# techpro-studio/NNToolkitCore

Hardware: AMD Instinct MI355X
Metric: audio frames/sec (whole node) (higher is better)
Workload: dtype f32

## Files before the change

### nntoolkitcore_amd/csrc/hip/nntk_common.hpp

```cpp
#pragma once
#include <hip/hip_runtime.h>
#include <math.h>
#include "nntk_shim.h"

hipStream_t nntk_stream();
int nntk_fail(const char *what, hipError_t err);
int nntk_fail_msg(const char *what);
enum { NNTK_SPAN_REC = 0, NNTK_SPAN_SPEC = 1 };
int nntk_prof_span_begin(int kind);
void nntk_prof_span_end(int idx, long launches, long units);

struct NntkOptions {
    int rec_persistent = -1;
    int rec_xw = -1;
    int rec_pingpong = -1;
    int rec_groups = 2;
    int rec_spin_us = 1000000;
    int rec_stream = -1;
    int rec_fused2 = -1;
    int rec_rr = -1;
    int rec_xf = -1;
    int rec_fk = -1;
    int rec_hf = -1;
    int rec_bd = -1;
    int dense_frag3 = -1;
    int dense_f16x2 = -1;
    int train_outer_plain = -1;
    int train_bptt = -1;
    int spec_ppw = 0;
    int spec_variant = -1;
#ifdef NNTK_VARIANT_SPEC_DMA
    int spec_dma = -1;
#endif
    int bn_fast = 0;
    int gemm_tm_batch = -1;
    int conv_a4 = 1;
    int conv_flatk = -1;
    int conv_frag3_out = -1;
    int conv_store = -1;
    int gemm_split_bf16 = -1;
    int gemm_wide = -1;
    int conv_dbg = 0;
    int weights_check = -1;
};
const NntkOptions &nntk_options();

unsigned *nntk_fault_word();
int nntk_fault_enqueue_copy();
int nntk_persistent_disabled();
void nntk_persistent_launch_begin();
void nntk_persistent_launch_end();
bool nntk_weights_exact_only(const void *d_wp);
int nntk_cu_count();
void nntk_set_last_conv_kernel(const char *name);
void nntk_set_last_rec_kernel(const char *name);
int nntk_set_max_dynamic_lds(const void *kernel, size_t bytes);
// ... 54 lines not shown
```

### nntoolkitcore_amd/csrc/hip/recurrent_rr.hip

```cpp
#include "recurrent_rr_common.hpp"

__host__ __device__ inline int rr_blocks_per_ct(int KH, int KX) { return 4 * KH * 2 * 2 + 4 * KH * 2 + 4 * KX * 2 * 3; }

template <bool RAW>
__global__ __launch_bounds__(256) void rr_pack_kernel(const float *__restrict__ ut, const float *__restrict__ wp,
                                                      rr_v4u *__restrict__ img, int H, int in, int Hj_p, int Hk_p, int Kin_p,
                                                      int KH, int KX, int NCT, float uscale = 0.0f, float wscale = 1.0f) {
    const int bpc = rr_blocks_per_ct(KH, KX);
    const long total = (long)NCT * bpc * 64;
    for (long e = blockIdx.x * (long)blockDim.x + threadIdx.x; e < total; e += (long)gridDim.x * blockDim.x) {
        const int l = (int)(e & 63);
        const long blk = e >> 6;
        const int ct = (int)(blk / bpc);
        int r = (int)(blk % bpc);
        int part, w, i, mt, m;
        const int n_uh = 4 * KH * 4, n_ul = 4 * KH * 2;
        if (r < n_uh) { part = 0; m = r & 1; mt = (r >> 1) & 1; i = (r >> 2) % KH; w = (r >> 2) / KH; }
        else if (r < n_uh + n_ul) { r -= n_uh; part = 1; m = 2; mt = r & 1; i = (r >> 1) % KH; w = (r >> 1) / KH; }
        else { r -= n_uh + n_ul; part = 2; m = r % 3; mt = (r / 3) & 1; i = (r / 6) % KX; w = (r / 6) / KX; }
        const int c = 32 * mt + (l & 31);
        const int g = (c >> 3) & 3;
        const int j = 16 * ct + 8 * ((c >> 2) & 1) + 4 * (c >> 5) + (c & 3);
        const int ks = part == 2 ? w * KX + i : w * KH + i;
        float v[8];
// ... 20 lines not shown
                for (int q = 0; q < 4; ++q) rr_split_pair_f16(v[2 * q] * uscale, v[2 * q + 1] * uscale, h4[q], l4[q]);
                img[e] = m == 0 ? (rr_v4u){h4[0], h4[1], h4[2], h4[3]} : (rr_v4u){l4[0], l4[1], l4[2], l4[3]};
                continue;
            }
            if (part == 1) { img[e] = (rr_v4u){0u, 0u, 0u, 0u}; continue; }
#pragma unroll
            for (int q = 0; q < 8; ++q) v[q] *= wscale;
        }
        rr_split8(v, hi, mid, lo);
        img[e] = m == 0 ? hi : m == 1 ? mid : lo;
    }
}

__global__ __launch_bounds__(256) void rr_tile_h0_kernel(const float *__restrict__ h0, rr_v4u *__restrict__ hb, int B, int H, int NKS) {
    const long total = (long)((B + 63) / 64) * 2 * (H / 16) * 64;
    for (long e = blockIdx.x * (long)blockDim.x + threadIdx.x; e < total; e += (long)gridDim.x * blockDim.x) {
        const int l = (int)(e & 63);
        long r = e >> 6;
        const int ks = (int)(r % (H / 16)); r /= (H / 16);
        const int half = (int)(r & 1);
        const long bt = r >> 1;
        const long row = bt * 64 + half * 32 + (l & 31);
        if (row >= B) continue;
        float v[8];
#pragma unroll
        for (int q = 0; q < 8; ++q) v[q] = h0[row * H + 16 * ks + 8 * (l >> 5) + q];
        rr_v4u hi, mid, lo;
        rr_split8(v, hi, mid, lo);
        rr_v4u *dst = hb + ((((size_t)bt * 2 + half) * NKS + ks) * 3) * 64 + l;
        dst[0] = hi; dst[64] = mid; dst[128] = lo;
    }
}

template <int KH, int KX, bool TRAIN, int CELL, bool XF, bool HF = false, bool VL = false, bool BD = false>
__device__ __forceinline__ void rr_body(const RRParams &p) {
    static_assert(!VL || !HF, "VL: not with the two-f16-image hand-off");
    static_assert(!BD || (VL && XF), "BD: per-row lengths and a frag3 x operand");
    constexpr int NH = HF ? 2 : 3;
#ifndef RR_ULR8
#define RR_ULR8 0
#endif
    constexpr bool ULR = !HF && (KX > 2 || (RR_ULR8 && KH == 8 && !TRAIN));
    constexpr int NST = KX + KH;
#ifndef RR_S_RED
#define RR_S_RED 0
#endif
    constexpr int S_RED = (RR_S_RED) && KH == 8 ? 1 : 0, S_PUB = S_RED + 1;
    constexpr int S_XSPL = KX > 2 ? KX : S_PUB + 1;
#ifndef RR_PEND
#define RR_PEND (KH == 4)
#endif
    constexpr bool PEND = RR_PEND;
#ifndef RR_S_E1_XLATE
#define RR_S_E1_XLATE 2
#endif
#ifndef RR_HF_S_E1
#define RR_HF_S_E1 2
#endif
    constexpr int S_E1 = (KX > 2 ? RR_S_E1_XLATE : HF ? RR_HF_S_E1 : RR_S_E1) + S_RED;
    constexpr bool X_LATE = KX > 2;
    constexpr int S_E2 = NST - 1;
#ifndef RR_HEAD_LEAD
#define RR_HEAD_LEAD 1
#endif
    constexpr int S_HEAD = !PEND ? S_E2 : S_E2 - RR_HEAD_LEAD > S_PUB ? S_E2 - RR_HEAD_LEAD : S_PUB + 1;
#ifndef RR_HF_NPRE
#define RR_HF_NPRE 5
#endif
    constexpr int NPRE = (HF ? RR_HF_NPRE : RR_NPRE) < KH ? (HF ? RR_HF_NPRE : RR_NPRE) : KH;
    constexpr int own_lo = S_PUB + NPRE < KH ? S_PUB + NPRE : KH, own_hi = S_E1 + NPRE < KH ? S_E1 + NPRE : KH;
    constexpr int NXR = XF ? 3 * KX : 2 * KX;
    constexpr int N_X_AFTER_PUB = (X_LATE || S_XSPL >= S_E1) ? 0 : NXR;
    constexpr int N_AFTER_PUB = NH * (own_hi - own_lo) + N_X_AFTER_PUB;
    static_assert(!HF || (!PEND && !TRAIN && XF && CELL == 0 && !ULR), "HF: the flag-protocol LSTM instantiations with a frag3 x operand");
    static_assert(NST >= 5 && S_XSPL >= KX && S_XSPL > S_PUB && KH - NPRE <= S_E2 && S_HEAD > S_PUB && S_HEAD <= S_E2, "slice schedule");
#ifndef RR_POLL_LEAD_RR
#define RR_POLL_LEAD_RR (NST >= 9 ? 2 : RR_POLL_LEAD)
#endif
#ifndef RR_HF_POLL_LEAD
#define RR_HF_POLL_LEAD RR_POLL_LEAD_RR
#endif
    constexpr int POLL_LEAD = HF ? RR_HF_POLL_LEAD : RR_POLL_LEAD_RR;
    static_assert(PEND ? S_XSPL < S_E2 : (S_E1 < S_E2 && S_E1 > S_PUB && S_XSPL < S_E2 - POLL_LEAD), "slice schedule");
    extern __shared__ __attribute__((aligned(16))) char smem[];
    rr_v4u *ULs = reinterpret_cast<rr_v4u *>(smem);
    rr_v4u *WXs = ULs + ((ULR || HF) ? 0 : 4 * KH * 2 * 64);
    rr_v4u *red = WXs + 4 * KX * 6 * 64;
    float *hx = reinterpret_cast<float *>(red + 32 * 64);
    unsigned *hs = reinterpret_cast<unsigned *>(hx + 32 * RR_HX_LD);

    const int tid = threadIdx.x;
    const int lane = tid & 63;
    const int w = __builtin_amdgcn_readfirstlane(tid >> 6);
    const int n = lane & 31, kh = lane >> 5;
    const int bt = blockIdx.x % p.NBT;
    const int ct = blockIdx.x / p.NBT;
    const int bt_abs = p.b_base / 64 + bt;
    const int b0 = p.b_base + bt * 64;
    const int H = p.H;
    const int T = VL ? __builtin_amdgcn_readfirstlane(p.len[p.B + bt_abs]) : p.T;
    const int NKS = H >> 4;
    const bool bwd = BD && b0 >= p.bd_pad;
    const int rb0 = bwd ? b0 - p.bd_pad : b0;
    const int rows_valid = BD ? (p.bd_rows - rb0 < 64 ? p.bd_rows - rb0 : 64) : p.B - b0 < 64 ? p.B - b0 : 64;
    if (VL && T == 0) {
        if constexpr (BD) rr_bd_pass_state(p, b0, 64, 16 * ct, 16);
        else rr_vl_pass_state(p, b0, 64, 16 * ct, 16, CELL == 0);
// ... 187 lines not shown
                const float zg = nntk_fast_sigmoid(zc[0][e]);
                const float rg = nntk_fast_sigmoid(zc[1][e]);
                const float ht = nntk_fast_tanh(fmaf(rg, zc[2][e], zc[3][e]));
                hn[e] = fmaf(-zg + 1.0f, ht, zg * cst[half][e]);
                if constexpr (VL) hn[e] = t < vlen[half] ? hn[e] : cst[half][e];
                cst[half][e] = hn[e];
                if (TRAIN) {
                    zc[2][e] = fmaf(rg, zc[2][e], zc[3][e]);
                    zc[3][e] = z[2][e] + bsum[2][e];
                    ac[0][e] = zg; ac[1][e] = rg; ac[2][e] = ht;
                }
                continue;
            }
            const float ig = nntk_fast_sigmoid(zc[0][e]);
            const float fg = nntk_fast_sigmoid(zc[1][e]);
            const float gg = nntk_fast_tanh(zc[2][e]);
            const float og = nntk_fast_sigmoid(zc[3][e]);
            const float cn = fmaf(fg, cst[half][e], ig * gg);
            if constexpr (VL) {
                const bool live = t < vlen[half];
                hn[e] = live ? og * nntk_fast_tanh(cn) : hkeep[half][e];
                cst[half][e] = live ? cn : cst[half][e];
                hkeep[half][e] = hn[e];
            } else {
            cst[half][e] = cn;
            hn[e] = og * nntk_fast_tanh(cn);
            }
            ac[0][e] = ig; ac[1][e] = fg; ac[2][e] = gg; ac[3][e] = og;
        }
        *reinterpret_cast<float2 *>(hx + n * RR_HX_LD + jl) = make_float2(hn[0], hn[1]);
        if (HF && !RR_DBG(128)) {
            unsigned sh, sl;
            rr_split_pair_h2(hn[0], hn[1], sh, sl);
            unsigned *d = hs + n * RR_HS_LD + (jl >> 1);
            d[0] = sh; d[32 * RR_HS_LD] = sl;
        } else if (!RR_DBG(128)) {
            unsigned sh, sm, sl;
            rr_split_pair(hn[0], hn[1], sh, sm, sl);
            if (PEND) { sh = min(sh, 0xfffffffeu); sm = min(sm, 0xfffffffeu); sl = min(sl, 0xfffffffeu); }
            unsigned *d = hs + n * RR_HS_LD + (jl >> 1);
            d[0] = sh; d[32 * RR_HS_LD] = sm; d[2 * 32 * RR_HS_LD] = sl;
        }
        bool own_step = true;
        if constexpr (VL) own_step = t < vlen[half];
        if (TRAIN && CELL == 1) {
            const int row = b0 + half * 32 + n;
            if (row < p.B && jf + 1 < H + 1 && own_step) {
                float *zrow = p.z_cache + ((size_t)row * p.T + t) * 6 * H + jf;
#pragma unroll
                for (int g = 0; g < 3; ++g) {
                    *reinterpret_cast<float2 *>(zrow + g * H) = make_float2(zc[g][0], zc[g][1]);
                    *reinterpret_cast<float2 *>(zrow + (3 + g) * H) = make_float2(ac[g][0], ac[g][1]);
                }
                *reinterpret_cast<float2 *>(p.c_cache + ((size_t)row * p.T + t) * H + jf) = make_float2(zc[3][0], zc[3][1]);
            }
        } else if (TRAIN) {
            const int row = b0 + half * 32 + n;
            if (row < p.B && jf + 1 < H + 1 && own_step) {
                float *zrow = p.z_cache + ((size_t)row * p.T + t) * 8 * H + jf;
#pragma unroll
                for (int g = 0; g < 4; ++g) {
                    *reinterpret_cast<float2 *>(zrow + g * H) = make_float2(zc[g][0], zc[g][1]);
                    *reinterpret_cast<float2 *>(zrow + (4 + g) * H) = make_float2(ac[g][0], ac[g][1]);
                }
                *reinterpret_cast<float2 *>(p.c_cache + ((size_t)row * p.T + t) * H + jf) = make_float2(cst[half][0], cst[half][1]);
            }
// ... 35 lines not shown
                rr_v4u h2hi, h2lo;
                rr_split8_h2(v8, h2hi, h2lo);
                const __amdgpu_buffer_rsrc_t rs2 = __builtin_amdgcn_make_buffer_rsrc((void *)(p.out_h2 + (size_t)t * p.h2step), 0, (int)p.h2step, 0x00020000);
                const int vo = lane16 + (((bt_abs * 2 + half) * NKS + ct) * 2) * 1024;
                __builtin_amdgcn_raw_buffer_store_b128(h2hi, rs2, vo, 0, 0);
                __builtin_amdgcn_raw_buffer_store_b128(h2lo, rs2, vo + 1024, 0, 0);
                RR_BOUND(5, (size_t)t * p.h2step, vo + 1024, 0, p.h2step, 16);
            }
            if (BD && LAST) {
                int b0e = rb0;
                asm volatile("" : "+s"(b0e));
                const int row = b0e + half * 32 + n;
                if (row < p.bd_rows && !p.return_sequences) {
                    float *o = (bwd ? p.out_b : p.out) + (size_t)row * ldo + 16 * ct + 8 * kh;
                    *reinterpret_cast<rr_v4u *>(o) = o0; *reinterpret_cast<rr_v4u *>(o + 4) = o1;
                }
            } else if (LAST) {
                int b0e = b0;
                asm volatile("" : "+s"(b0e));
                const int row = b0e + half * 32 + n;
                if (row < p.B) {
                    if (!p.return_sequences && p.out) {
                        float *o = p.out + (size_t)row * H + 16 * ct + 8 * kh;
                        *reinterpret_cast<rr_v4u *>(o) = o0; *reinterpret_cast<rr_v4u *>(o + 4) = o1;
                    }
                    if (p.hT) {
                        float *o = p.hT + (size_t)row * H + 16 * ct + 8 * kh;
                        *reinterpret_cast<rr_v4u *>(o) = o0; *reinterpret_cast<rr_v4u *>(o + 4) = o1;
                    }
                }
            }
        } else if (PEND && w == ((2 * half + 2) & 3)) {
            if (!RR_DBG(128)) {
                const int vo = lane16 + (((bt_abs * 2 + half) * NKS + ct) * 3) * 1024;
                const __amdgpu_buffer_rsrc_t rs2 = rs_wr(t + 2 < T ? t + 2 : t);
                const int vo2 = t + 2 < T ? vo : RR_OOB_F;
                const rr_v4u pend = {RR_PENDING, RR_PENDING, RR_PENDING, RR_PENDING};
                __builtin_amdgcn_raw_buffer_store_b128(pend, rs2, vo2, 0, RR_ST_AUX);
                __builtin_amdgcn_raw_buffer_store_b128(pend, rs2, vo2 + 1024, 0, RR_ST_AUX);
                __builtin_amdgcn_raw_buffer_store_b128(pend, rs2, vo2 + 2048, 0, RR_ST_AUX);
                RR_BOUND(3, (size_t)(t + 2 < T ? t + 2 : t) * p.hstep, vo2 + 2048, 0, hb_bytes, 16);
            }
        }
    };
    unsigned *const flags0 = p.flags + (size_t)bt * 2 * RR_FLAGS, *const flags1 = flags0 + RR_FLAGS;
    auto arrive = [&](int half, int t, auto xlive_tag) __attribute__((always_inline)) {
        if (w == 2 * half) {
            asm volatile("s_waitcnt vmcnt(%0)" :: "i"(N_AFTER_PUB - (decltype(xlive_tag)::value ? 0 : N_X_AFTER_PUB)) : "memory");
            if (lane == 0)
                __hip_atomic_store((half ? flags1 : flags0) + ct, (unsigned)(t + 1), __ATOMIC_RELAXED, __HIP_MEMORY_SCOPE_AGENT);
        }
    };
    unsigned pv0 = 0;
    const bool flag_live = lane < p.NCT;
    auto poll_a = [&](int half) __attribute__((always_inline)) {
        const unsigned *f = (half ? flags1 : flags0) + lane;
        asm volatile("global_load_dword %0, %1, off sc1" : "=v"(pv0) : "v"(f) : "memory");
    };
    auto poll_b = [&](int half, int t) __attribute__((always_inline)) {
        asm volatile("s_waitcnt vmcnt(0)" : "+v"(pv0) :: "memory");
        const unsigned target = (unsigned)t;
        bool ok = !flag_live || pv0 >= target;
        if (__builtin_amdgcn_ballot_w64(!ok) != 0 || p.spin_ticks == 0) {
            const unsigned *f = (half ? flags1 : flags0) + lane;
            const unsigned long long t_start = __builtin_amdgcn_s_memrealtime();
            bool expired = p.spin_ticks == 0;
            while (!expired) {
                const unsigned a = __hip_atomic_load(f, __ATOMIC_RELAXED, __HIP_MEMORY_SCOPE_AGENT);
                ok = !flag_live || a >= target;
                if (__builtin_amdgcn_ballot_w64(!ok) == 0) break;
                if (__hip_atomic_load(p.fault, __ATOMIC_RELAXED, __HIP_MEMORY_SCOPE_AGENT) != 0) { expired = true; break; }
                __builtin_amdgcn_s_sleep(1);
                expired = __builtin_amdgcn_s_memrealtime() - t_start > p.spin_ticks;
            }
            if (expired && lane == 0) __hip_atomic_fetch_or(p.fault, 1u, __ATOMIC_RELAXED, __HIP_MEMORY_SCOPE_AGENT);
        }
    };

    auto probe_h = [&](auto half_tag, int i) __attribute__((always_inline)) {
        constexpr int half = decltype(half_tag)::value;
        unsigned mx = 0;
#pragma unroll
        for (int m = 0; m < 3; ++m) {
            const rr_v4u v = hf[half][i][m];
            mx = max(mx, max(max(v.x, v.y), max(v.z, v.w)));
        }
        return __builtin_amdgcn_ballot_w64(mx == RR_PENDING);
    };
    const unsigned long long inject = p.spin_ticks == 0 ? ~0ull : 0ull;
    auto settle_h = [&](auto half_tag, int t, int i, unsigned long long pend) __attribute__((always_inline)) {
        if (__builtin_expect((pend | inject) != 0, 0)) {
            const unsigned long long t_start = __builtin_amdgcn_s_memrealtime();
            bool expired = p.spin_ticks == 0;
            while (!expired) {
                issue_h(half_tag, t, 3 * i, 3 * i + 3);
                if (probe_h(half_tag, i) == 0) break;
                if (__hip_atomic_load(p.fault, __ATOMIC_RELAXED, __HIP_MEMORY_SCOPE_AGENT) != 0) { expired = true; break; }
                __builtin_amdgcn_s_sleep(1);
                expired = __builtin_amdgcn_s_memrealtime() - t_start > p.spin_ticks;
            }
            if (expired && lane == 0) __hip_atomic_fetch_or(p.fault, 1u, __ATOMIC_RELAXED, __HIP_MEMORY_SCOPE_AGENT);
        }
    };

    auto exchange = [&](const f32x16 (&acc)[2], int d0, int d1) __attribute__((always_inline)) {
        if (RR_DBG(32)) return;
#pragma unroll
        for (int dst = 0; dst < 4; ++dst) {
            if (dst < d0 || dst >= d1) continue;
            const int mt = dst >> 1, o = 2 * (dst & 1);
            const rr_v4u q0 = {__float_as_uint(acc[mt][o]), __float_as_uint(acc[mt][o + 1]), __float_as_uint(acc[mt][4 + o]), __float_as_uint(acc[mt][5 + o])};
            const rr_v4u q1 = {__float_as_uint(acc[mt][8 + o]), __float_as_uint(acc[mt][9 + o]), __float_as_uint(acc[mt][12 + o]), __float_as_uint(acc[mt][13 + o])};
            red[((dst * 4 + w) * 2 + 0) * 64 + lane] = q0;
            red[((dst * 4 + w) * 2 + 1) * 64 + lane] = q1;
        }
    };
    auto half_step = [&](auto y_tag, auto fin_tag, auto next_tag, auto poll_tag, auto last_tag, auto xlive_tag, int t, int tX) __attribute__((always_inline)) {
        constexpr bool XLIVE = decltype(xlive_tag)::value;
        constexpr int Y = decltype(y_tag)::value;
        using XT = std::integral_constant<int, 1 - Y>;
        constexpr int X = 1 - Y;
        constexpr bool FIN = decltype(fin_tag)::value, NEXT = decltype(next_tag)::value, POLL = decltype(poll_tag)::value;
        constexpr bool YCHK = PEND;
        f32x16 acc[2];
        unsigned long long pend_next = 0;
#pragma unroll
        for (int mt = 0; mt < 2; ++mt)
#pragma unroll
// ... 8 lines not shown
                for (int mt = 0; mt < 2; ++mt)
#pragma unroll
                    for (int m = 0; m < 3; ++m)
                        wa[mt][m] = __builtin_bit_cast(rr_bf16x8, WXs[((((w * KX + s) * 2 + mt) * 3) + m) * 64 + lane]);
            } else if (ULR) {
#pragma unroll
                for (int mt = 0; mt < 2; ++mt) ulo[mt] = ulr[s - KX][mt];
            } else if (HF) {
            } else {
#pragma unroll
                for (int mt = 0; mt < 2; ++mt)
                    ulo[mt] = ULPRE ? ulo_n[mt]
                                    : __builtin_bit_cast(rr_bf16x8, ULs[((w * KH + (s - KX)) * 2 + mt) * 64 + lane]);
            }
            if (s == S_RED && FIN && !RR_DBG(2)) { fin_reduce(); fin_gates(XT{}, tX); }
            if (s == S_PUB && FIN && !RR_DBG(2)) { fin_publish(XT{}, last_tag, tX); }
            if (!PEND) {
                if (s == S_E1 && FIN && !RR_DBG(4)) { arrive(X, tX, xlive_tag); }
                if (s == S_E2 - POLL_LEAD && NEXT && POLL && !RR_DBG(4)) poll_a(X);
                if (s == S_E2 && NEXT && POLL && !RR_DBG(4)) poll_b(X, tX + 1);
            }
            if (s == S_HEAD && NEXT && !RR_DBG(1)) issue_h(XT{}, tX + 1, 0, NH * NPRE);
            if (s == S_E2 && X_LATE && XLIVE && !RR_DBG(8)) issue_x(y_tag, t + 1);
            if (s + NPRE < KH && !RR_DBG(1)) issue_h(y_tag, t, NH * (s + NPRE), NH * (s + NPRE + 1));
            if (RR_DBG(16)) {
            } else if (s < KX) {
#pragma unroll
                for (int pr = 0; pr < 6; ++pr)
#pragma unroll
                    for (int mt = 0; mt < 2; ++mt)
                        acc[mt] = __builtin_amdgcn_mfma_f32_32x32x16_bf16(wa[mt][PA[pr]], xf[XF ? Y : 0][s][PB[pr]], acc[mt], 0, 0, 0);
            } else {
                const int i = s - KX;
                if (YCHK && t > 0 && !RR_DBG(4) && !RR_DBG(1)) settle_h(y_tag, t, i, pend_next);
                if constexpr (HF) {
                    constexpr int QA[3] = {0, 1, 0}, QB[3] = {1, 0, 0};
                    rr_f16x8 bh[2];
#pragma unroll
                    for (int m = 0; m < 2; ++m) bh[m] = __builtin_bit_cast(rr_f16x8, hf[Y][i][m]);
                    if (s == NST - 1) {
#pragma unroll
                        for (int mt = 0; mt < 2; ++mt) {
#pragma unroll
                            for (int pr = 0; pr < 3; ++pr)
                                acc[mt] = __builtin_amdgcn_mfma_f32_32x32x16_f16(__builtin_bit_cast(rr_f16x8, uh[i][mt][QA[pr]]), bh[QB[pr]], acc[mt], 0, 0, 0);
                            if (mt == 0) exchange(acc, 0, 2);
                        }
                    } else {
#pragma unroll
                        for (int pr = 0; pr < 3; ++pr)
#pragma unroll
                            for (int mt = 0; mt < 2; ++mt)
                                acc[mt] = __builtin_amdgcn_mfma_f32_32x32x16_f16(__builtin_bit_cast(rr_f16x8, uh[i][mt][QA[pr]]), bh[QB[pr]], acc[mt], 0, 0, 0);
                    }
                } else {
                rr_bf16x8 b[3];
#pragma unroll
                for (int m = 0; m < 3; ++m) b[m] = __builtin_bit_cast(rr_bf16x8, hf[Y][i][m]);
                if (s == NST - 1) {
#pragma unroll
                    for (int mt = 0; mt < 2; ++mt) {
#pragma unroll
                        for (int pr = 0; pr < 6; ++pr) {
                            const rr_bf16x8 av = PA[pr] == 2 ? ulo[mt] : uh[i][mt][PA[pr]];
                            acc[mt] = __builtin_amdgcn_mfma_f32_32x32x16_bf16(av, b[PB[pr]], acc[mt], 0, 0, 0);
                        }
                        if (mt == 0) exchange(acc, 0, 2);
                    }
                } else {
#pragma unroll
                for (int pr = 0; pr < 6; ++pr)
#pragma unroll
                    for (int mt = 0; mt < 2; ++mt) {
                        const rr_bf16x8 av = PA[pr] == 2 ? ulo[mt] : uh[i][mt][PA[pr]];
                        acc[mt] = __builtin_amdgcn_mfma_f32_32x32x16_bf16(av, b[PB[pr]], acc[mt], 0, 0, 0);
                    }
                }
                }
            }
            if (YCHK && s + 1 >= KX && s + 1 < NST && !RR_DBG(4) && !RR_DBG(1)) pend_next = probe_h(y_tag, s + 1 - KX);
            if (ULPRE && s + 1 >= KX && s + 1 < NST) {
#pragma unroll
                for (int mt = 0; mt < 2; ++mt) ulo_n[mt] = __builtin_bit_cast(rr_bf16x8, ULs[((w * KH + (s + 1 - KX)) * 2 + mt) * 64 + lane]);
            }
            if (s == S_XSPL) {
                if (NEXT && !RR_DBG(8)) split_x();
                if (!X_LATE && XLIVE && !RR_DBG(8)) issue_x(y_tag, t + 1);
            }
#ifndef RR_NO_INTERLEAVE
#ifdef RR_VALU_IL
#pragma unroll
            for (int j = 0; j < 12; ++j) {
                __builtin_amdgcn_sched_group_barrier(0x008, 1, 0);
                __builtin_amdgcn_sched_group_barrier(0x002, RR_VALU_IL, 0);
                if (j & 1) __builtin_amdgcn_sched_group_barrier(0x010, 1, 0);
            }
#else
            if (s == NST - 1) {
#pragma unroll
                for (int j = 0; j < 3; ++j) {
                    __builtin_amdgcn_sched_group_barrier(0x008, 2, 0);
                    __builtin_amdgcn_sched_group_barrier(0x010, 1, 0);
                }
#pragma unroll
                for (int j = 0; j < 4; ++j) {
                    __builtin_amdgcn_sched_group_barrier(0x008, 1, 0);
                    __builtin_amdgcn_sched_group_barrier(0x200, 1, 0);
                    __builtin_amdgcn_sched_group_barrier(0x010, 1, 0);
                }
                __builtin_amdgcn_sched_group_barrier(0x008, 2, 0);
            } else {
#pragma unroll
            for (int j = 0; j < 6; ++j) {
// ... 9 lines not shown
        exchange(acc, 2, 4);
    };

    issue_x(I0{}, 0);
    issue_h(I0{}, 0, 0, NH * NPRE);
    split_x();
    issue_x(I1{}, 0);
    if (T > 1) {
        half_step(I0{}, Ff{}, Tt{}, Ff{}, Ff{}, Tt{}, 0, -1);
        half_step(I1{}, Tt{}, Tt{}, Tt{}, Ff{}, Tt{}, 0, 0);
        for (int t = 1; t < T - 1; ++t) {
            half_step(I0{}, Tt{}, Tt{}, Tt{}, Ff{}, Tt{}, t, t - 1);
            half_step(I1{}, Tt{}, Tt{}, Tt{}, Ff{}, Tt{}, t, t);
        }
        half_step(I0{}, Tt{}, Tt{}, Tt{}, Ff{}, Ff{}, T - 1, T - 2);
    } else {
        half_step(I0{}, Ff{}, Tt{}, Ff{}, Ff{}, Ff{}, 0, -1);
    }
    half_step(I1{}, Tt{}, Ff{}, Ff{}, Tt{}, Ff{}, T - 1, T - 1);
    fin_reduce();
    fin_gates(I1{}, T - 1);
    fin_publish(I1{}, Tt{}, T - 1);
    int b0e = b0;
    asm volatile("" : "+s"(b0e));
#pragma unroll
    for (int half = 0; half < 2; ++half) {
        const int row = b0e + half * 32 + n;
        if (p.cT && row < p.B) {
            if (jf < H) p.cT[(size_t)row * H + jf] = cst[half][0];
            if (jf + 1 < H) p.cT[(size_t)row * H + jf + 1] = cst[half][1];
        }
    }
}
template <int KH, int KX, bool TRAIN = false, bool XF = false, bool HF = false, bool VL = false, bool BD = false>
__global__ __launch_bounds__(256) void lstm_rr_kernel(RRParams p) { rr_body<KH, KX, TRAIN, 0, XF, HF, VL, BD>(p); }
template <int KH, int KX, bool TRAIN = false, bool XF = false, bool VL = false, bool BD = false>
__global__ __launch_bounds__(256) void gru_rr_kernel(RRParams p) { rr_body<KH, KX, TRAIN, 1, XF, false, VL, BD>(p); }

#ifdef NNTK_RR_BOUNDS
static unsigned long long *g_rr_bounds = nullptr;
extern "C" int nntk_shim_rr_bounds_fetch(unsigned long long out[8]) {
    for (int i = 0; i < 8; ++i) out[i] = 0;
    if (!g_rr_bounds) return 0;
    if (hipDeviceSynchronize() != hipSuccess) return -1;
    if (hipMemcpy(out, g_rr_bounds, 64, hipMemcpyDeviceToHost) != hipSuccess) return -1;
    (void)hipMemset(g_rr_bounds, 0, 64);
    return 0;
}
#endif
static bool rr_shape(int H, int in, bool xf, int *KH, int *KX) {
    if (H < 64 || H > 512 || (H % 16) != 0 || in < 1) return false;
    if (!xf && (in < 8 || (in % 8) != 0)) return false;
    *KH = H <= 256 ? 4 : 8;
    *KX = in <= 64 ? 1 : in <= 128 ? 2 : (in <= 256 && *KH == 4) ? 4 : 0;
    return *KX != 0;
}
static bool rr_shape_hf(int H, int in, int *KH, int *KX) {
    if (H <= 256 || H > 512 || (H % 16) != 0 || in < 1) return false;
    *KH = 8;
    *KX = in <= 64 ? 1 : in <= 128 ? 2 : in <= 256 ? 4 : 0;
    return *KX != 0;
}
static size_t rr_lds_bytes(int KH, int KX, bool train = false, bool hf = false) {
    const bool ulr = hf || KX > 2 || (RR_ULR8 && KH == 8 && !train);
    return (size_t)((ulr ? 0 : 4 * KH * 2) + 4 * KX * 6 + 32) * 1024 + 32 * RR_HX_LD * 4 + 3 * 32 * RR_HS_LD * 4;
}
static size_t rr_step_bytes(int B, int H) { return (size_t)((B + 63) / 64) * 2 * (H / 16) * 3 * 1024; }

// ... 153 lines not shown
}

static int rr_launch(const RRIo &io, const float *d_img, const float *d_bi, const float *d_bh,
                     int B, int T, int in, int H, int return_sequences, int cell) {
    if (B <= 0 || T <= 0) return 0;
    const bool xf = io.xf3 != nullptr;
    const bool train = io.c_cache != nullptr;
    if (xf && (train || io.x_tm)) return 1;
    const bool vl = io.len != nullptr;
    if (vl && (io.x_tm || io.out_tm || io.hf || io.out_h2)) return nntk_fail_msg("lstm_rr: lengths with a stacked / frag2h call");
    const bool bd = io.out_b != nullptr;
    if (bd && (!vl || !xf || io.h0 || io.hT || io.cT)) return nntk_fail_msg("lstm_rr: a bidirectional call needs lengths, a frag3 x and no carried state");
    if (!xf && !io.x) return nntk_fail_msg("lstm_rr: no input");
    if (!io.hseq || !io.work) return nntk_fail_msg("lstm_rr: no hand-off buffer");
    if (io.x_tm && (double)T * B * in * 4 >= 2.0e9) return 1;
    if (io.out_tm && (!return_sequences || !io.out || (double)T * B * H * 4 >= 2.0e9)) return 1;
    if (io.out_h2 && (io.out || io.img4 || train || !return_sequences)) return nntk_fail_msg("lstm_rr: frag2h output with an f32 output / on the full-K family");
    const NntkOptions &opt = nntk_options();
    if (opt.rec_rr == 0 || opt.rec_persistent == 0 || nntk_persistent_disabled()) return 1;
    int KH, KX;
    const bool hf = io.hf != 0;
    if (!(hf ? rr_shape_hf(H, in, &KH, &KX) : rr_shape(H, in, xf, &KH, &KX))) return 1;
    if (!xf && ((((size_t)io.x) & 15) != 0 || (in % 4) != 0)) return 1;
    if (hf && (KH != 8 || cell != 0 || !xf || train || io.h0 || io.out || io.out_h2 || io.img4 || !return_sequences || opt.rec_hf == 0)) return 1;
    const int NCT = H / 16;
    if (!rr_tile_fits(T, in, bd ? io.ldo : H)) return 1;
    void (*kern)(RRParams) = nullptr;
    if (KH == 8 && KX == 2) kern = rr_pick<8, 2>(cell, train, xf, vl, bd);
    else if (KH == 8 && KX == 1) kern = rr_pick<8, 1>(cell, train, xf, vl, bd);
    else if (KH == 4 && KX == 4) kern = rr_pick<4, 4>(cell, train, xf, vl, bd);
    else if (KH == 4 && KX == 2) kern = rr_pick<4, 2>(cell, train, xf, vl, bd);
    else if (KH == 4 && KX == 1) kern = rr_pick<4, 1>(cell, train, xf, vl, bd);
    if (hf) kern = KX == 4 ? lstm_rr_kernel<8, 4, false, true, true> : KX == 2 ? lstm_rr_kernel<8, 2, false, true, true> : lstm_rr_kernel<8, 1, false, true, true>;
    if (!kern) return 1;
    const size_t lds = rr_lds_bytes(KH, KX, train, hf);
    if (lds > 160 * 1024) return 1;
    if (nntk_set_max_dynamic_lds((const void *)kern, lds)) return -1;
    const int resident = nntk_resident_blocks((const void *)kern, 256, lds, 1);
    const int tiles_per_launch = resident / NCT;
    if (tiles_per_launch < 1) return 1;
    unsigned *fault = nntk_fault_word();
    if (!fault) return 1;
    const size_t step = hf ? rr_step_bytes(B, H) / 3 * 2 : rr_step_bytes(B, H);
    if (step >= (size_t)RR_OOB_F) return 1;
    const int nbt_total = (B + 63) / 64;
    const size_t xstep = (size_t)nbt_total * 2 * ((in + 15) / 16) * 3 * 1024;
    if (xf && xstep >= (size_t)RR_OOB_F) return 1;
    unsigned *flags = reinterpret_cast<unsigned *>(io.work + step / 4);
    if (nntk_shim_memset(io.work, 0, step + (size_t)((B + 127) / 128) * 4 * RR_FLAGS * sizeof(unsigned))) return -1;
    if (nntk_shim_memset(io.hseq, 0xff, step * (size_t)(T < 2 ? T : 2))) return -1;
    if (io.h0) {
        long g = ((long)nbt_total * 2 * NCT * 64 + 255) / 256;
        if (g > 2048) g = 2048;
        hipLaunchKernelGGL(rr_tile_h0_kernel, dim3((unsigned)g), dim3(256), 0, nntk_stream(), io.h0, (rr_v4u *)io.work, B, H, H / 16);
    }
    RRParams q;
    q.x = io.x; q.img = (const rr_v4u *)d_img; q.bi = d_bi; q.bh = d_bh;
    q.h0f = (char *)io.work; q.hseq = (char *)io.hseq; q.hstep = step;
    q.xf3 = (const char *)io.xf3; q.xstep = xstep; q.NKSx = (in + 15) / 16;
    q.c0 = io.c0; q.cT = io.cT; q.hT = io.hT; q.out = io.out;
    q.c_cache = io.c_cache; q.z_cache = io.z_cache;
    q.x_tm = io.x_tm; q.out_tm = io.out_tm;
    q.fault = fault;
    q.spin_ticks = (unsigned long long)(opt.rec_spin_us > 0 ? opt.rec_spin_us : 0) * 100ull;
    q.B = B; q.T = T; q.H = H; q.in = in; q.NCT = NCT; q.return_sequences = return_sequences;
    q.NHT = nbt_total * 2;
    q.out_h2 = (char *)io.out_h2; q.h2step = rr_step_bytes(B, H) / 3 * 2;
    q.z_scale = io.z_scale;
    q.len = io.len; q.h0 = io.h0;
    q.img_b = (const rr_v4u *)io.img_b; q.bi_b = io.bi_b; q.bh_b = io.bh_b; q.out_b = io.out_b;
    q.bd_pad = bd ? B / 2 : 0; q.bd_rows = io.bd_rows; q.ldo = io.ldo;
#ifdef NNTK_REC_STAMPS
    q.stamp = nullptr;
    const char *stamp_path = getenv("NNTK_REC_STAMP_FILE");
    if (stamp_path) {
        if (hipMalloc((void **)&q.stamp, (size_t)(T + 1) * 64 * 8) != hipSuccess) return nntk_fail_msg("stamp alloc");
        (void)hipMemset(q.stamp, 0, (size_t)(T + 1) * 64 * 8);
    }
#endif
#ifdef NNTK_RR_BOUNDS
    static unsigned long long *g_bounds = nullptr;
    if (!g_bounds) {
// ... 9 lines not shown
    int took4 = 1;
    if (xf && !train && io.img4 && !io.out_tm) {
        q.flags = flags;
        took4 = nntk_fk_launch(q, io.img4, io.img4_b, cell, &launches);
        if (took4 < 0) { nntk_persistent_launch_end(); return -1; }
    }
    if (took4 == 1)
    for (int bt0 = 0; bt0 < nbt_total; bt0 += tiles_per_launch) {
        const int nbt = nbt_total - bt0 < tiles_per_launch ? nbt_total - bt0 : tiles_per_launch;
        q.NBT = nbt; q.b_base = bt0 * 64;
        q.flags = flags + (size_t)bt0 * 2 * RR_FLAGS;
        hipLaunchKernelGGL(kern, dim3((unsigned)(nbt * NCT)), dim3(256), lds, nntk_stream(), q);
    }
    const int copy_rc = nntk_fault_enqueue_copy();
    nntk_persistent_launch_end();
    if (copy_rc) return -1;
    nntk_prof_span_end(span, (long)launches, T);
#ifdef NNTK_REC_STAMPS
    if (q.stamp) {
        (void)hipStreamSynchronize(nntk_stream());
        unsigned long long *hs = (unsigned long long *)malloc((size_t)(T + 1) * 64 * 8);
        (void)hipMemcpy(hs, q.stamp, (size_t)(T + 1) * 64 * 8, hipMemcpyDeviceToHost);
        FILE *f = fopen(stamp_path, "wb");
        if (f) { fwrite(hs, 8, (size_t)(T + 1) * 64, f); fclose(f); }
        free(hs); (void)hipFree(q.stamp);
    }
#endif
    NNTK_LAUNCH_CHECK("lstm_rr_kernel");
    static const char *const names[2][2][3] = {{{"lstm_rr_kernel<4,1>", "lstm_rr_kernel<4,2>", "lstm_rr_kernel<4,4>"}, {"lstm_rr_kernel<8,1>", "lstm_rr_kernel<8,2>", ""}},
                                               {{"gru_rr_kernel<4,1>", "gru_rr_kernel<4,2>", "gru_rr_kernel<4,4>"}, {"gru_rr_kernel<8,1>", "gru_rr_kernel<8,2>", ""}}};
    static const char *const bd_names[2][2][3] = {{{"lstm_rr_kernel<4,1,bd>", "lstm_rr_kernel<4,2,bd>", "lstm_rr_kernel<4,4,bd>"}, {"lstm_rr_kernel<8,1,bd>", "lstm_rr_kernel<8,2,bd>", ""}},
                                                  {{"gru_rr_kernel<4,1,bd>", "gru_rr_kernel<4,2,bd>", "gru_rr_kernel<4,4,bd>"}, {"gru_rr_kernel<8,1,bd>", "gru_rr_kernel<8,2,bd>", ""}}};
    if (bd && took4 == 1) nntk_set_last_rec_kernel(bd_names[cell == 1][KH == 8][KX == 1 ? 0 : KX == 2 ? 1 : 2]);
    else if (hf) nntk_set_last_rec_kernel(KX == 4 ? "lstm_rr_kernel<8,4,hf>" : KX == 2 ? "lstm_rr_kernel<8,2,hf>" : "lstm_rr_kernel<8,1,hf>");
    else if (took4 == 1) nntk_set_last_rec_kernel(names[cell == 1][KH == 8][KX == 1 ? 0 : KX == 2 ? 1 : 2]);
    return 0;
}
```

### nntoolkitcore_amd/csrc/hip/runtime.hip

```cpp
#include "nntk_common.hpp"
#include <stdio.h>
#include <string.h>
#include <vector>

#include <atomic>
#include <mutex>
#include <stdlib.h>

static thread_local hipStream_t t_stream = nullptr;
static thread_local char g_err[512] = "";

hipStream_t nntk_stream() { return t_stream; }

int nntk_fail(const char *what, hipError_t err) {
    snprintf(g_err, sizeof(g_err), "HIP error in %s: %s", what, hipGetErrorString(err));
    return -1;
}
int nntk_fail_msg(const char *what) {
    snprintf(g_err, sizeof(g_err), "%s", what);
    return -1;
}

static NntkOptions g_opt;
static std::once_flag g_opt_once;
static std::mutex g_opt_mutex;

struct OptDesc { const char *name; const char *env; int NntkOptions::*field; };
static const OptDesc g_opt_table[] = {
    {"rec_persistent", "NNTK_REC_PERSISTENT", &NntkOptions::rec_persistent},
    {"rec_xw", "NNTK_REC_XW", &NntkOptions::rec_xw},
    {"rec_pingpong", "NNTK_REC_PINGPONG", &NntkOptions::rec_pingpong},
    {"rec_groups", "NNTK_REC_GROUPS", &NntkOptions::rec_groups},
    {"rec_spin_us", "NNTK_REC_SPIN_US", &NntkOptions::rec_spin_us},
    {"rec_stream", "NNTK_REC_STREAM", &NntkOptions::rec_stream},
    {"rec_fused2", "NNTK_REC_FUSED2", &NntkOptions::rec_fused2},
    {"rec_rr", "NNTK_REC_RR", &NntkOptions::rec_rr},
    {"rec_xf", "NNTK_REC_XF", &NntkOptions::rec_xf},
    {"rec_fk", "NNTK_REC_FK", &NntkOptions::rec_fk},
    {"rec_hf", "NNTK_REC_HF", &NntkOptions::rec_hf},
    {"rec_bd", "NNTK_REC_BD", &NntkOptions::rec_bd},
    {"dense_frag3", "NNTK_DENSE_FRAG3", &NntkOptions::dense_frag3},
    {"dense_f16x2", "NNTK_DENSE_F16X2", &NntkOptions::dense_f16x2},
    {"train_bptt", "NNTK_TRAIN_BPTT", &NntkOptions::train_bptt},
    {"train_outer_plain", "NNTK_TRAIN_OUTER_PLAIN", &NntkOptions::train_outer_plain},
    {"spec_ppw", "NNTK_SPEC_PPW", &NntkOptions::spec_ppw},
    {"spec_variant", "NNTK_SPEC_VARIANT", &NntkOptions::spec_variant},
#ifdef NNTK_VARIANT_SPEC_DMA
    {"spec_dma", "NNTK_SPEC_DMA", &NntkOptions::spec_dma},
#endif
    {"bn_fast", "NNTK_BN_FAST", &NntkOptions::bn_fast},
    {"gemm_tm_batch", "NNTK_GEMM_TM_BATCH", &NntkOptions::gemm_tm_batch},
    {"gemm_split_bf16", "NNTK_GEMM_SPLIT_BF16", &NntkOptions::gemm_split_bf16},
    {"conv_store", "NNTK_CONV_STORE", &NntkOptions::conv_store},
    {"conv_frag3_out", "NNTK_CONV_FRAG3_OUT", &NntkOptions::conv_frag3_out},
    {"conv_flatk", "NNTK_CONV_FLATK", &NntkOptions::conv_flatk},
    {"conv_a4", "NNTK_CONV_A4", &NntkOptions::conv_a4},
    {"gemm_wide", "NNTK_GEMM_WIDE", &NntkOptions::gemm_wide},
    {"conv_dbg", "NNTK_CONV_DBG", &NntkOptions::conv_dbg},
    {"weights_check", "NNTK_WEIGHTS_CHECK", &NntkOptions::weights_check},
};
static void opt_init() {
    for (const OptDesc &d : g_opt_table) {
        const char *e = getenv(d.env);
        if (e && *e && strcmp(e, "auto") != 0 && strcmp(e, "default") != 0) g_opt.*(d.field) = atoi(e);
    }
}
const NntkOptions &nntk_options() {
    std::call_once(g_opt_once, opt_init);
    return g_opt;
}

struct ProfSpan { hipEvent_t a, b; long launches, units; int kind; hipStream_t stream; };
// ... 625 lines not shown
```

### nntoolkitcore_amd/csrc/host/recurrent.c

```c
#include <stdarg.h>
#include <stdio.h>
#include <math.h>
#include <stdlib.h>
#include <string.h>
#include <time.h>
#include "nntk_internal.h"

#define NNTK_STREAM_MAX_T 32

RecurrentConfig RecurrentConfigCreate(int input_feature_channels, int output_feature_channels,
                                      bool return_sequences, int timesteps) {
    RecurrentConfig c;
    memset(&c, 0, sizeof(c));
    c.input_feature_channels = input_feature_channels;
    c.output_feature_channels = output_feature_channels;
    c.return_sequences = return_sequences;
    c.timesteps = timesteps;
    return c;
}


typedef struct {
    int G;
    int in, H, T;
    bool return_sequences;
    RecurrentWeights *weights;
    nntk_wblock wb;
    float *d_wp, *d_bi, *d_ut, *d_bh;
    float *d_wt;
    int wt_valid;
    int rr_exact_only;
    float *d_rr4;
    float *d_rr;
    int rr_valid;
    float *d_rr_hf;
    int rr_hf_valid;
    float hf_wscale;
    float *d_b4, *d_b4_train;
    float *d_rr_train;
    float *d_h[2], *d_c[2];
    int cur;
    float *pin_in, *pin_out;
    size_t pin_in_n, pin_out_n;
    unsigned *d_done;
    volatile unsigned *flag;
    unsigned seq;
    nntk_devbuf d_in, d_out, d_xw, d_work, d_work_rr, d_rr_stage;
    nntk_devbuf d_h2;
    nntk_devbuf d_hseq;
    nntk_devbuf d_xf3;
    nntk_devbuf d_len;
    nntk_devbuf d_bd, d_bd_len;
} rec_core;

typedef struct {
    int on, mini_batch, have_batch;
    const float *d_x_cur;
    nntk_devbuf d_x, d_h, d_Zg, d_hU, d_dxW, d_dhU, d_work, d_raw, d_grad, d_scr, d_dout, d_dX;
    nntk_train_vl vl;
    nntk_devbuf d_len, d_xm;
    nntk_devbuf d_s0;
    nntk_devbuf d_st;
    nntk_devbuf d_yo;
    float *want_hT, *want_cT;
} rec_train;

typedef struct {
    rec_core core;
    rec_train train;
    int use_bh;
// ... 122 lines not shown
    if (!l) return;
    core_free(&l->core);
    train_free(&l->train);
    free(l);
}

static float *pack_gate_transposed(const float *src, int G, int H, size_t *n) {
    const int Hj_p = (H + 15) & ~15, Hk_p = (H + 31) & ~31;
    *n = (size_t)G * Hj_p * Hk_p;
    float *tmp = (float *)calloc(*n, sizeof(float));
    if (!tmp) { nntk_set_error("out of host memory while packing recurrent weights"); return NULL; }
    for (int k = 0; k < H; ++k)
        for (int g = 0; g < G; ++g)
            for (int j = 0; j < H; ++j)
                tmp[((size_t)g * Hj_p + j) * Hk_p + k] = src[(size_t)k * G * H + (size_t)g * H + j];
    return tmp;
}

static int core_upload(rec_core *c) {
    int G = c->G, H = c->H;
    if (nntk_upload_gemm_weights(&c->d_wp, c->weights->W, c->in, G * H)) return -1;
    if (nntk_upload_floats(&c->d_bi, c->weights->b_i, (size_t)G * H)) return -1;
    if (nntk_upload_floats(&c->d_bh, c->weights->b_h, (size_t)G * H)) return -1;
    size_t n;
    float *tmp = pack_gate_transposed(c->weights->U, G, H, &n);
    if (!tmp) return -1;
    int rc = nntk_upload_floats(&c->d_ut, tmp, n);
    free(tmp);
    if (rc) return rc;
    c->wt_valid = 0;
    c->rr_valid = 0;
    c->rr_hf_valid = 0;
    c->rr_exact_only = rr_unsplittable(c->weights->W, (size_t)c->in * G * H + (size_t)H * G * H);
    nntk_wblock_mark_uploaded(&c->wb);
    return 0;
}

static int core_ensure_wt(rec_core *c) {
    if (c->wt_valid) return 0;
    if (c->in != c->H) NNTK_FAIL("fused GRU stack: layer 2's input size must equal its hidden size");
    size_t n;
    float *tmp = pack_gate_transposed(c->weights->W, c->G, c->H, &n);
    if (!tmp) return -1;
    int rc = nntk_upload_floats(&c->d_wt, tmp, n);
    free(tmp);
    if (rc) return rc;
    c->wt_valid = 1;
    return 0;
}

static int core_ensure(rec_core *c, int check_edits) {
    if (nntk_wblock_dirty(&c->wb, check_edits)) return core_upload(c);
    return 0;
}

static int core_reset_state(rec_core *c) {
    size_t hs = ((size_t)c->H + 63) & ~(size_t)63;
    c->cur = 0;
    return nntk_shim_memset(c->d_h[0], 0, 4 * hs * sizeof(float));
}

static int core_broadcast(rec_core *c, int root) {
    if (nntk_shim_dist_broadcast_host(c->wb.host, c->wb.n, root)) return -1;
    return core_upload(c);
}
static int core_sync(rec_core *c) {
// ... 1169 lines not shown
    return layer_apply_batch(&filter->l, input, output, batch);
}
int LSTMApplyDevice(LSTM filter, const float *d_input, float *d_output, int batch) {
    REC_ENTER("LSTMApplyDevice", filter);
    return layer_apply_device(&filter->l, d_input, d_output, batch);
}
int LSTMApplyDeviceVarLen(LSTM filter, const float *d_input, float *d_output, int batch, const int *lengths,
                          const float *d_h0, const float *d_c0, float *d_hT, float *d_cT) {
    REC_ENTER("LSTMApplyDeviceVarLen", filter);
    return layer_apply_device_vl(&filter->l, "LSTMApplyDeviceVarLen", d_input, d_output, batch, lengths, d_h0, d_c0, d_hT, d_cT);
}
int LSTMApplyInferenceBatchVarLen(LSTM filter, const float *input, float *output, int batch, const int *lengths,
                                  const float *h0, const float *c0, float *hT, float *cT) {
    REC_ENTER("LSTMApplyInferenceBatchVarLen", filter);
    return layer_apply_host_vl(&filter->l, "LSTMApplyInferenceBatchVarLen", input, output, batch, lengths, h0, c0, hT, cT);
}
int LSTMApplyDeviceFrag3(LSTM filter, const float *d_input, const float *d_input_frag3, float *d_output, float *d_output_frag3, int batch) {
    REC_ENTER("LSTMApplyDeviceFrag3", filter);
    return layer_apply_device_f3(&filter->l, d_input, d_input_frag3, d_output, d_output_frag3, batch);
}
int LSTMBidirectionalApplyDevice(LSTM forward, LSTM backward, const float *d_input, float *d_output, int batch, const int *lengths, int merge) {
    REC_ENTER("LSTMBidirectionalApplyDevice", forward && backward);
    return layer_apply_bd(&forward->l, &backward->l, "LSTMBidirectionalApplyDevice", d_input, d_output, batch, lengths, merge);
}
int LSTMBidirectionalApplyInferenceBatch(LSTM forward, LSTM backward, const float *input, float *output, int batch, const int *lengths, int merge) {
    REC_ENTER("LSTMBidirectionalApplyInferenceBatch", forward && backward);
    return layer_apply_bd_host(&forward->l, &backward->l, "LSTMBidirectionalApplyInferenceBatch", input, output, batch, lengths, merge);
}

static int lstm_try_rr_hf(rec_layer *l, const float *d_in, const float *d_in_f3, float *d_out_h2, int B) {
    rec_core *c = &l->core;
    if (rr_why_not(l, c->rr_exact_only, nntk_shim_lstm_rr_hf_ok(c->H, c->in))) return 1;
    if (!c->rr_hf_valid) {
        const size_t nW = (size_t)c->in * 4 * c->H, nU = (size_t)c->H * 4 * c->H;
        float us = nntk_f16_scale(c->weights->U, nU), mw = 0.f;
        for (size_t i = 0; i < nW; ++i) { float a = fabsf(c->weights->W[i]); if (a > mw) mw = a; }
        c->hf_wscale = (us > 0.f && us < 1e15f && us > 1e-15f && mw * 32768.f * us < 1e30f) ? 32768.f * us : 0.f;
        if (c->hf_wscale > 0.f) {
            size_t img = nntk_shim_lstm_rr_hf_image_floats(c->H, c->in);
            if (!c->d_rr_hf && !(c->d_rr_hf = (float *)nntk_shim_malloc(img * sizeof(float)))) return -1;
            if (nntk_shim_lstm_rr_pack_hf(c->d_ut, c->d_wp, c->d_rr_hf, c->H, c->in, us, c->hf_wscale)) return -1;
        }
        c->rr_hf_valid = 1;
    }
    if (!(c->hf_wscale > 0.f)) return 1;
    const float *xf3 = d_in_f3;
    if (!xf3) {
        float *buf = nntk_devbuf_reserve(&c->d_xf3, nntk_shim_frag3_floats(B, c->T, c->in));
        if (!buf || nntk_shim_frag3_pack(d_in, buf, B, c->T, c->in)) return -1;
        xf3 = buf;
    }
    float *d_work = nntk_devbuf_reserve(&c->d_work_rr, nntk_shim_lstm_rr_work_floats(B, c->H));
    if (!d_work) return -1;
    return nntk_shim_lstm_rr_hf(xf3, c->d_rr_hf, c->d_bi, l->use_bh ? c->d_bh : NULL, d_out_h2, d_work, B, c->T, c->in, c->H, 1.f / c->hf_wscale);
}
static int lstm_apply_device_h2(LSTM filter, const float *d_in, const float *d_in_f3, float *d_out_h2, int B) {
    rec_layer *l = &filter->l;
    rec_core *c = &l->core;
    if (layer_acts(l)) return -1;
    if (!layer_std_acts(l) || !c->return_sequences) return 1;
    if (B <= 0 || c->T <= 0) return 0;
    if (core_ensure(c, 0)) return -1;
    int rc = lstm_try_rr_hf(l, d_in, d_in_f3, d_out_h2, B);
    if (rc <= 0) return rc;
    if (!nntk_shim_fk_image_floats(c->H, c->in)) {
        const rr_io io = { .d_in = d_in, .d_in_f3 = d_in_f3, .d_out_h2 = d_out_h2 };
        rc = core_try_rr(l, &io, B, 0);
        if (rc <= 0) return rc;
    }
    float *o = nntk_devbuf_reserve(&c->d_out, (size_t)B * c->T * c->H);
    if (!o) return -1;
    if (core_apply_device_f3(l, d_in, d_in_f3, o, NULL, B)) return -1;
    return nntk_shim_frag2h_pack(o, d_out_h2, B, c->T, c->H);
}
// ... 164 lines not shown
```

Measured before the change: 74.53 million.

## Use pending-sentinel handoff instead of flags for HF LSTM recurrent kernel

Adds an HP instantiation of the two-f16-image LSTM recurrent kernel (KX=1,2) that detects arrival of the hidden-state slices with the pending-sentinel pattern, replacing the separate flag protocol. Published values are clamped below the sentinel, only two pending stores are written per slice, and the flag memset is skipped. It also sets a separate head lead for HF and moves the f16 scale computation from the first apply to weight upload. The aim is lower per-step synchronisation latency on the recurrent critical path, at the risk of extra polling traffic and a rare value clamp.

```diff
diff --git a/nntoolkitcore_amd/csrc/hip/nntk_common.hpp b/nntoolkitcore_amd/csrc/hip/nntk_common.hpp
--- a/nntoolkitcore_amd/csrc/hip/nntk_common.hpp
+++ b/nntoolkitcore_amd/csrc/hip/nntk_common.hpp
@@ -22,6 +22,7 @@
     int rec_xf = -1;
     int rec_fk = -1;
     int rec_hf = -1;
+    int rec_hf_pend = 1;
     int rec_bd = -1;
     int dense_frag3 = -1;
     int dense_f16x2 = -1;
diff --git a/nntoolkitcore_amd/csrc/hip/recurrent_rr.hip b/nntoolkitcore_amd/csrc/hip/recurrent_rr.hip
--- a/nntoolkitcore_amd/csrc/hip/recurrent_rr.hip
+++ b/nntoolkitcore_amd/csrc/hip/recurrent_rr.hip
@@ -76,9 +76,10 @@
     }
 }
 
-template <int KH, int KX, bool TRAIN, int CELL, bool XF, bool HF = false, bool VL = false, bool BD = false>
+template <int KH, int KX, bool TRAIN, int CELL, bool XF, bool HF = false, bool VL = false, bool BD = false, bool HP = false>
 __device__ __forceinline__ void rr_body(const RRParams &p) {
     static_assert(!VL || !HF, "VL: not with the two-f16-image hand-off");
+    static_assert(!HP || HF, "HP: the pending-pattern form of the HF instantiations");
     static_assert(!BD || (VL && XF), "BD: per-row lengths and a frag3 x operand");
     constexpr int NH = HF ? 2 : 3;
 #ifndef RR_ULR8
@@ -94,7 +95,7 @@
 #ifndef RR_PEND
 #define RR_PEND (KH == 4)
 #endif
-    constexpr bool PEND = RR_PEND;
+    constexpr bool PEND = RR_PEND || HP;
 #ifndef RR_S_E1_XLATE
 #define RR_S_E1_XLATE 2
 #endif
@@ -107,7 +108,11 @@
 #ifndef RR_HEAD_LEAD
 #define RR_HEAD_LEAD 1
 #endif
-    constexpr int S_HEAD = !PEND ? S_E2 : S_E2 - RR_HEAD_LEAD > S_PUB ? S_E2 - RR_HEAD_LEAD : S_PUB + 1;
+#ifndef RR_HF_HEAD_LEAD
+#define RR_HF_HEAD_LEAD 2
+#endif
+    constexpr int HEAD_LEAD = HF ? RR_HF_HEAD_LEAD : RR_HEAD_LEAD;
+    constexpr int S_HEAD = !PEND ? S_E2 : S_E2 - HEAD_LEAD > S_PUB ? S_E2 - HEAD_LEAD : S_PUB + 1;
 #ifndef RR_HF_NPRE
 #define RR_HF_NPRE 5
 #endif
@@ -116,7 +121,7 @@
     constexpr int NXR = XF ? 3 * KX : 2 * KX;
     constexpr int N_X_AFTER_PUB = (X_LATE || S_XSPL >= S_E1) ? 0 : NXR;
     constexpr int N_AFTER_PUB = NH * (own_hi - own_lo) + N_X_AFTER_PUB;
-    static_assert(!HF || (!PEND && !TRAIN && XF && CELL == 0 && !ULR), "HF: the flag-protocol LSTM instantiations with a frag3 x operand");
+    static_assert(!HF || (PEND == HP && !TRAIN && XF && CELL == 0 && !ULR), "HF: the LSTM instantiations with a frag3 x operand, on flags or (HP) the pending pattern");
     static_assert(NST >= 5 && S_XSPL >= KX && S_XSPL > S_PUB && KH - NPRE <= S_E2 && S_HEAD > S_PUB && S_HEAD <= S_E2, "slice schedule");
 #ifndef RR_POLL_LEAD_RR
 #define RR_POLL_LEAD_RR (NST >= 9 ? 2 : RR_POLL_LEAD)
@@ -370,6 +375,7 @@
         if (HF && !RR_DBG(128)) {
             unsigned sh, sl;
             rr_split_pair_h2(hn[0], hn[1], sh, sl);
+            if (PEND) { sh = min(sh, 0xfffffffeu); sl = min(sl, 0xfffffffeu); }
             unsigned *d = hs + n * RR_HS_LD + (jl >> 1);
             d[0] = sh; d[32 * RR_HS_LD] = sl;
         } else if (!RR_DBG(128)) {
@@ -471,14 +477,14 @@
             }
         } else if (PEND && w == ((2 * half + 2) & 3)) {
             if (!RR_DBG(128)) {
-                const int vo = lane16 + (((bt_abs * 2 + half) * NKS + ct) * 3) * 1024;
+                const int vo = lane16 + (((bt_abs * 2 + half) * NKS + ct) * NH) * 1024;
                 const __amdgpu_buffer_rsrc_t rs2 = rs_wr(t + 2 < T ? t + 2 : t);
                 const int vo2 = t + 2 < T ? vo : RR_OOB_F;
                 const rr_v4u pend = {RR_PENDING, RR_PENDING, RR_PENDING, RR_PENDING};
                 __builtin_amdgcn_raw_buffer_store_b128(pend, rs2, vo2, 0, RR_ST_AUX);
                 __builtin_amdgcn_raw_buffer_store_b128(pend, rs2, vo2 + 1024, 0, RR_ST_AUX);
-                __builtin_amdgcn_raw_buffer_store_b128(pend, rs2, vo2 + 2048, 0, RR_ST_AUX);
-                RR_BOUND(3, (size_t)(t + 2 < T ? t + 2 : t) * p.hstep, vo2 + 2048, 0, hb_bytes, 16);
+                if (!HF) __builtin_amdgcn_raw_buffer_store_b128(pend, rs2, vo2 + 2048, 0, RR_ST_AUX);
+                RR_BOUND(3, (size_t)(t + 2 < T ? t + 2 : t) * p.hstep, vo2 + (NH - 1) * 1024, 0, hb_bytes, 16);
             }
         }
     };
@@ -520,7 +526,7 @@
         constexpr int half = decltype(half_tag)::value;
         unsigned mx = 0;
 #pragma unroll
-        for (int m = 0; m < 3; ++m) {
+        for (int m = 0; m < NH; ++m) {
             const rr_v4u v = hf[half][i][m];
             mx = max(mx, max(max(v.x, v.y), max(v.z, v.w)));
         }
@@ -532,7 +538,7 @@
             const unsigned long long t_start = __builtin_amdgcn_s_memrealtime();
             bool expired = p.spin_ticks == 0;
             while (!expired) {
-                issue_h(half_tag, t, 3 * i, 3 * i + 3);
+                issue_h(half_tag, t, NH * i, NH * i + NH);
                 if (probe_h(half_tag, i) == 0) break;
                 if (__hip_atomic_load(p.fault, __ATOMIC_RELAXED, __HIP_MEMORY_SCOPE_AGENT) != 0) { expired = true; break; }
                 __builtin_amdgcn_s_sleep(1);
@@ -607,7 +613,9 @@
                         acc[mt] = __builtin_amdgcn_mfma_f32_32x32x16_bf16(wa[mt][PA[pr]], xf[XF ? Y : 0][s][PB[pr]], acc[mt], 0, 0, 0);
             } else {
                 const int i = s - KX;
-                if (YCHK && t > 0 && !RR_DBG(4) && !RR_DBG(1)) settle_h(y_tag, t, i, pend_next);
+                if constexpr (YCHK) {
+                    if (t > 0 && !RR_DBG(4) && !RR_DBG(1)) settle_h(y_tag, t, i, pend_next);
+                }
                 if constexpr (HF) {
                     constexpr int QA[3] = {0, 1, 0}, QB[3] = {1, 0, 0};
                     rr_f16x8 bh[2];
@@ -653,7 +661,9 @@
                 }
                 }
             }
-            if (YCHK && s + 1 >= KX && s + 1 < NST && !RR_DBG(4) && !RR_DBG(1)) pend_next = probe_h(y_tag, s + 1 - KX);
+            if constexpr (YCHK) {
+                if (s + 1 >= KX && s + 1 < NST && !RR_DBG(4) && !RR_DBG(1)) pend_next = probe_h(y_tag, s + 1 - KX);
+            }
             if (ULPRE && s + 1 >= KX && s + 1 < NST) {
 #pragma unroll
                 for (int mt = 0; mt < 2; ++mt) ulo_n[mt] = __builtin_bit_cast(rr_bf16x8, ULs[((w * KH + (s + 1 - KX)) * 2 + mt) * 64 + lane]);
@@ -729,8 +739,8 @@
         }
     }
 }
-template <int KH, int KX, bool TRAIN = false, bool XF = false, bool HF = false, bool VL = false, bool BD = false>
-__global__ __launch_bounds__(256) void lstm_rr_kernel(RRParams p) { rr_body<KH, KX, TRAIN, 0, XF, HF, VL, BD>(p); }
+template <int KH, int KX, bool TRAIN = false, bool XF = false, bool HF = false, bool VL = false, bool BD = false, bool HP = false>
+__global__ __launch_bounds__(256) void lstm_rr_kernel(RRParams p) { rr_body<KH, KX, TRAIN, 0, XF, HF, VL, BD, HP>(p); }
 template <int KH, int KX, bool TRAIN = false, bool XF = false, bool VL = false, bool BD = false>
 __global__ __launch_bounds__(256) void gru_rr_kernel(RRParams p) { rr_body<KH, KX, TRAIN, 1, XF, false, VL, BD>(p); }
 
@@ -950,6 +960,8 @@
     else if (KH == 4 && KX == 2) kern = rr_pick<4, 2>(cell, train, xf, vl, bd);
     else if (KH == 4 && KX == 1) kern = rr_pick<4, 1>(cell, train, xf, vl, bd);
     if (hf) kern = KX == 4 ? lstm_rr_kernel<8, 4, false, true, true> : KX == 2 ? lstm_rr_kernel<8, 2, false, true, true> : lstm_rr_kernel<8, 1, false, true, true>;
+    const bool hp = hf && KX != 4 && opt.rec_hf_pend != 0;
+    if (hp) kern = KX == 2 ? lstm_rr_kernel<8, 2, false, true, true, false, false, true> : lstm_rr_kernel<8, 1, false, true, true, false, false, true>;
     if (!kern) return 1;
     const size_t lds = rr_lds_bytes(KH, KX, train, hf);
     if (lds > 160 * 1024) return 1;
@@ -965,7 +977,7 @@
     const size_t xstep = (size_t)nbt_total * 2 * ((in + 15) / 16) * 3 * 1024;
     if (xf && xstep >= (size_t)RR_OOB_F) return 1;
     unsigned *flags = reinterpret_cast<unsigned *>(io.work + step / 4);
-    if (nntk_shim_memset(io.work, 0, step + (size_t)((B + 127) / 128) * 4 * RR_FLAGS * sizeof(unsigned))) return -1;
+    if (nntk_shim_memset(io.work, 0, step + (hp ? 0 : (size_t)((B + 127) / 128) * 4 * RR_FLAGS * sizeof(unsigned)))) return -1;
     if (nntk_shim_memset(io.hseq, 0xff, step * (size_t)(T < 2 ? T : 2))) return -1;
     if (io.h0) {
         long g = ((long)nbt_total * 2 * NCT * 64 + 255) / 256;
@@ -1041,6 +1053,9 @@
     static const char *const bd_names[2][2][3] = {{{"lstm_rr_kernel<4,1,bd>", "lstm_rr_kernel<4,2,bd>", "lstm_rr_kernel<4,4,bd>"}, {"lstm_rr_kernel<8,1,bd>", "lstm_rr_kernel<8,2,bd>", ""}},
                                                   {{"gru_rr_kernel<4,1,bd>", "gru_rr_kernel<4,2,bd>", "gru_rr_kernel<4,4,bd>"}, {"gru_rr_kernel<8,1,bd>", "gru_rr_kernel<8,2,bd>", ""}}};
     if (bd && took4 == 1) nntk_set_last_rec_kernel(bd_names[cell == 1][KH == 8][KX == 1 ? 0 : KX == 2 ? 1 : 2]);
+    else if (hf && KX != 4 && hp != (NntkOptions().rec_hf_pend != 0))
+        nntk_set_last_rec_kernel(hp ? (KX == 2 ? "lstm_rr_kernel<8,2,pend,hf>" : "lstm_rr_kernel<8,1,pend,hf>")
+                                    : (KX == 2 ? "lstm_rr_kernel<8,2,flags,hf>" : "lstm_rr_kernel<8,1,flags,hf>"));
     else if (hf) nntk_set_last_rec_kernel(KX == 4 ? "lstm_rr_kernel<8,4,hf>" : KX == 2 ? "lstm_rr_kernel<8,2,hf>" : "lstm_rr_kernel<8,1,hf>");
     else if (took4 == 1) nntk_set_last_rec_kernel(names[cell == 1][KH == 8][KX == 1 ? 0 : KX == 2 ? 1 : 2]);
     return 0;
diff --git a/nntoolkitcore_amd/csrc/hip/runtime.hip b/nntoolkitcore_amd/csrc/hip/runtime.hip
--- a/nntoolkitcore_amd/csrc/hip/runtime.hip
+++ b/nntoolkitcore_amd/csrc/hip/runtime.hip
@@ -38,6 +38,7 @@
     {"rec_xf", "NNTK_REC_XF", &NntkOptions::rec_xf},
     {"rec_fk", "NNTK_REC_FK", &NntkOptions::rec_fk},
     {"rec_hf", "NNTK_REC_HF", &NntkOptions::rec_hf},
+    {"rec_hf_pend", "NNTK_REC_HF_PEND", &NntkOptions::rec_hf_pend},
     {"rec_bd", "NNTK_REC_BD", &NntkOptions::rec_bd},
     {"dense_frag3", "NNTK_DENSE_FRAG3", &NntkOptions::dense_frag3},
     {"dense_f16x2", "NNTK_DENSE_F16X2", &NntkOptions::dense_f16x2},
diff --git a/nntoolkitcore_amd/csrc/host/recurrent.c b/nntoolkitcore_amd/csrc/host/recurrent.c
--- a/nntoolkitcore_amd/csrc/host/recurrent.c
+++ b/nntoolkitcore_amd/csrc/host/recurrent.c
@@ -35,7 +35,7 @@
     int rr_valid;
     float *d_rr_hf;
     int rr_hf_valid;
-    float hf_wscale;
+    float hf_uscale, hf_wscale;
     float *d_b4, *d_b4_train;
     float *d_rr_train;
     float *d_h[2], *d_c[2];
@@ -224,6 +224,13 @@
     c->rr_valid = 0;
     c->rr_hf_valid = 0;
     c->rr_exact_only = rr_unsplittable(c->weights->W, (size_t)c->in * G * H + (size_t)H * G * H);
+    c->hf_uscale = c->hf_wscale = 0.f;
+    if (G == 4 && H > 256 && H <= 512) {
+        const size_t nW = (size_t)c->in * 4 * H, nU = (size_t)H * 4 * H;
+        float us = nntk_f16_scale(c->weights->U, nU), mw = 0.f;
+        for (size_t i = 0; i < nW; ++i) { float a = fabsf(c->weights->W[i]); if (a > mw) mw = a; }
+        if (us > 0.f && us < 1e15f && us > 1e-15f && mw * 32768.f * us < 1e30f) { c->hf_uscale = us; c->hf_wscale = 32768.f * us; }
+    }
     nntk_wblock_mark_uploaded(&c->wb);
     return 0;
 }
@@ -1459,14 +1466,10 @@
     rec_core *c = &l->core;
     if (rr_why_not(l, c->rr_exact_only, nntk_shim_lstm_rr_hf_ok(c->H, c->in))) return 1;
     if (!c->rr_hf_valid) {
-        const size_t nW = (size_t)c->in * 4 * c->H, nU = (size_t)c->H * 4 * c->H;
-        float us = nntk_f16_scale(c->weights->U, nU), mw = 0.f;
-        for (size_t i = 0; i < nW; ++i) { float a = fabsf(c->weights->W[i]); if (a > mw) mw = a; }
-        c->hf_wscale = (us > 0.f && us < 1e15f && us > 1e-15f && mw * 32768.f * us < 1e30f) ? 32768.f * us : 0.f;
         if (c->hf_wscale > 0.f) {
             size_t img = nntk_shim_lstm_rr_hf_image_floats(c->H, c->in);
             if (!c->d_rr_hf && !(c->d_rr_hf = (float *)nntk_shim_malloc(img * sizeof(float)))) return -1;
-            if (nntk_shim_lstm_rr_pack_hf(c->d_ut, c->d_wp, c->d_rr_hf, c->H, c->in, us, c->hf_wscale)) return -1;
+            if (nntk_shim_lstm_rr_pack_hf(c->d_ut, c->d_wp, c->d_rr_hf, c->H, c->in, c->hf_uscale, c->hf_wscale)) return -1;
         }
         c->rr_hf_valid = 1;
     }
```

Result: no change. 74.50 million (median of 2 runs) (-0.0%).
